# bernardomig/torch_semantic_segmentation

Hardware: AMD Instinct MI355X
Metric: images/sec (train step) fastscnn 1024x2048 bs=8 (higher is better)
Workload: dtype bf16; 1 GPU; fastscnn train step (zero_grad+fwd+CE(ignore 255)+bwd+AdamW), 8 x 3 x 1024 x 2048 per GPU, 19 classes, random-init weights; global_batch=8, parallelism=dp1, hip_graph=True, syncbn=False

## Files before the change

include/tss_hip.h:

```cpp
#ifndef TSS_HIP_H
#define TSS_HIP_H

#ifdef __cplusplus
extern "C" {
#endif

#define TSS_OK 0
#define TSS_ERR_DTYPE (-1)
#define TSS_ERR_SHAPE (-2)
#define TSS_ERR_ALIGN (-3)
#define TSS_ERR_HIP (-4)

#define TSS_F32 0
#define TSS_BF16 1

typedef struct tss_bn_bwd_job {
  const double* bstats; double count; const float* invstd; const float* gamma; int training; int accumulate;
  float* dgamma; float* dbeta; float* ga; float* gb; float* gce; int C;
  int xchg_world; int xchg_rank; void* xchg_peers[8]; void* xchg_counters;
} tss_bn_bwd_job;

enum {
  TSS_K_PWCONV_FWD = 0, TSS_K_PWCONV_BWD_DATA, TSS_K_PWCONV_BWD_WEIGHT,
  TSS_K_CONV3X3_FWD, TSS_K_CONV3X3_BWD_DATA, TSS_K_CONV3X3_BWD_WEIGHT,
// ... 158 lines not shown
int tss_mul_addrows_bwd(const void* g, long ldg, const void* u, long ldu, const void* a, long lda, void* du, long lddu, void* da,
                        long ldda, void* dr, long lddr, float* ws, int B, long HW, int C, int dtype, void* stream);
int tss_scale_rows(const void* x, long ldx, const float* m, void* out, long ldo, int B, long HW, int C, int dtype, void* stream);
int tss_cat2_add(const void* gl, long ldl, const void* gr, long ldr, const void* gs, long lds, void* out, long ldo, long P, int half,
                 int dtype, void* stream);
int tss_pad_channels(const void* g, long ldg, int C, void* out, long ldo, int CP, long P, int dtype, void* stream);
int tss_ssnbt_tail_fwd(const void* left, long ldl, const float* mean_l, const float* scale_l, const float* shift_l,
                       const void* right, long ldr, const float* mean_r, const float* scale_r, const float* shift_r,
                       const void* x, long ldx, const float* m, void* out, long ldo, int B, long HW, int C, int dtype, void* stream);
int tss_ssnbt_tail_bwd(const void* dout, long lddo, const void* out, long ldo,
                       const void* left, long ldl, const float* mean_l, const void* right, long ldr, const float* mean_r,
                       const float* m, void* e, long lde, void* gs, long ldgs, double* stats_l, double* stats_r,
                       int B, long HW, int C, int dtype, void* stream);

int tss_channel_shuffle(const void* x, long ldx, void* y, long ldy, long P, int C, int groups, int dtype, void* stream);

int tss_stem3x3_fwd(const void* x_nchw, int x_is_f32, const float* w, void* y, long ldy, double* stats,
                    int B, int Cin, int Hin, int Win, int N, int stride, int dtype, void* stream);
int tss_stem3x3_bwd_weight(const void* e, long lde, const void* yraw, long ldyr,
                           const float* ga, const float* gb, const float* gce, const float* gmu,
                           const void* x_nchw, int x_is_f32, float* dw,
                           float* ws ,
                           int B, int Cin, int Hin, int Win, int N, int stride, int dtype, void* stream);

int tss_dwconv3x3_fwd(const void* x, long ldx, const float* in_mean, const float* in_scale, const float* in_bias, int in_relu,
                      const float* w, void* y, long ldy, double* stats,
                      int B, int Hin, int Win, int C, int stride, int dil, int dtype, void* stream);
int tss_dwconv3x3_bwd_data(const void* e, long lde, const void* yraw, long ldyr,
                           const float* ga, const float* gb, const float* gce, const float* gmu, const float* w,
                           const void* xraw, long ldx, const float* in_mean, const float* in_scale, const float* in_bias, int in_relu,
                           void* e_in, long ldei, double* bstats, const float* wg_ws, float* wg_dw,
                           int B, int Hin, int Win, int C, int stride, int dil, int dtype, void* stream);
int tss_pwconv_bwd_data_radd_supported(long P, int K, int N, int dtype);
int tss_pwconv_bwd_data_joined(const void* e, long lde, const void* yraw, long ldyr,
                               const float* ga, const float* gb, const float* gce, const float* gmu, const float* w, const void* wT_bf16,
                               void* e_in, long ldei, const float* wg_ws, float* wg_dw, long wg_P, int wg_K, int wg_N,
                               const void* radd, long ldr, const void* join_out, long ldjo, const void* join_y, long ldjy,
                               const float* join_mean, double* join_bstats, long P, int K, int N, int dtype, void* stream);
int tss_pwconv_bwd_data_radd(const void* e, long lde, const void* yraw, long ldyr,
                             const float* ga, const float* gb, const float* gce, const float* gmu, const float* w, const void* wT_bf16,
                             void* e_in, long ldei, const float* wg_ws, float* wg_dw, long wg_P, int wg_K, int wg_N,
                             const void* radd, long ldr, long P, int K, int N, int dtype, void* stream);
int tss_pwconv_bwd_fused_preferred(long P, int Cin, int Cout, int dtype);
int tss_pwconv_bwd_fused_rows(long P, int Cin, int Cout);
int tss_pwconv_bwd_fused(const void* e, long lde, const void* yraw, long ldyr, const float* ga, const float* gb, const float* gce,
                         const float* gmu, const float* w, const void* wT_bf16, const void* x, long ldx, const float* in_mean,
// ... 270 lines not shown
```

torch_semantic_segmentation_amd/csrc/prof.cpp:

```cpp
#include <mutex>
#include <vector>

#include "common.h"

namespace {

struct KernelInfo { const char* name; const char* symbol; };
const KernelInfo kInfo[TSS_K_COUNT] = {
    {"pwconv_fwd", "pwfast_kernel<false>|pwfast_mc_kernel<false>|convgemm_kernel"},
    {"pwconv_bwd_data", "pwfast_kernel<true>|pwfast_mc_kernel<true>|pwbwd_kernel|pwsweep_kernel|convgemm_kernel"},
    {"pwconv_bwd_weight", "wgfast_kernel|wgrad_kernel"},
    {"conv3x3_fwd", "conv3x3_wstat_kernel|conv3x3_stream_kernel|conv3x3_lean_kernel<false>|fc1d_kernel|convgemm_kernel<fwd>"}, {"conv3x3_bwd_data", "conv3x3_lean_kernel<true>|fc1d_kernel|convgemm_kernel<bwd>"}, {"conv3x3_bwd_weight", "fc1d_wgrad_kernel|wgrad_kernel"},
    {"stem3x3_fwd", "stem_fwd_mfma_kernel|convgemm_kernel"}, {"stem3x3_bwd_weight", "stem_wgrad_mfma_kernel|stem_wgrad_kernel"},
    {"dwconv3x3_fwd", "dw_fwd_roll_kernel|dw_fwd_strip_kernel"}, {"dwconv3x3_bwd_data", "dw_bwd_roll_s1_kernel|dw_bwd_roll_s2_kernel|dw_bwd_data_strip_kernel"},
    {"dwconv3x3_bwd_weight", "dw_bwd_weight_strip_kernel"},
    {"bn_finalize", "bn_finalize_kernel"}, {"bn_bwd_finalize", "bn_bwd_finalize_kernel"},
    {"join_fwd", "join_fwd_kernel"}, {"join_bwd", "join_bwd_kernel"},
    {"dropout", "dropout_kernel"}, {"bias_grad", "colsum_kernel"}, {"adamw", "adamw_kernel"},
    {"bilinear_nhwc_fwd", "bilinear_nhwc_fwd_kernel|ppm_concat_fwd_kernel"}, {"bilinear_nhwc_bwd_rows", "bilinear_nhwc_bwd_rows_kernel|ppm_concat_bwd_kernel"},
    {"bilinear_nhwc_bwd_cols", "bilinear_nhwc_bwd_cols_kernel"},
    {"bilinear_planar_fwd", "bilinear_planar_fwd_kernel"},
    {"upsample_head_fwd", "upsample_head_fwd_kernel"}, {"upsample_head_bwd_rows", "upsample_head_bwd_rows_kernel"},
    {"upsample_head_bwd_cols", "upsample_head_bwd_cols_kernel"},
    {"adaptive_pool_fwd", "adaptive_pool_fwd_kernel|ppm_pool_fwd_kernel"}, {"adaptive_pool_bwd", "adaptive_pool_bwd_kernel|ppm_pool_bwd_kernel"},
    {"copy_nhwc", "copy_nhwc_kernel"},
    {"cross_entropy_fwd", "ce_fwd_kernel"}, {"cross_entropy_bwd", "ce_bwd_kernel"}, {"argmax_confusion", "argmax_confusion_kernel"},
    {"upsample_ce_fwd", "upsample_ce_onepass_kernel"}, {"upsample_ce_bwd", "upsample_ce_gather_kernel"},
    {"resize_flip_planar", "resize_flip_planar_kernel"}, {"multiscale_argmax_confusion", "multiscale_argmax_kernel"},
    {"sgd", "sgd_kernel"}, {"grad_norm", "grad_sqnorm_kernel|grad_sqnorm_final_kernel"},
    {"upsample_ce_wide_fwd", "wide_ce_kernel"}, {"upsample_ce_wide_bwd", "wide_ce_gather_kernel"},
    {"argmax_confusion_wide", "wide_upsample_argmax_kernel|wide_planar_argmax_kernel"},
    {"multiscale_argmax_confusion_wide", "wide_multiscale_argmax_kernel"},
};

struct Rec { int kid; hipEvent_t a, b; double bytes, flops; };
struct Total { long launches; double ms, bytes, flops; };
// ... 116 lines not shown
```

torch_semantic_segmentation_amd/csrc/stem.hip:

```cpp
#include "common.h"

namespace {

constexpr int NT = 256;

struct StemArgs {
  const void* x; int x_f32;
  const float* w; void* y; long ldy; double* stats;
  int B, Cin, Hin, Win, Hout, Wout, N, stride;
};

struct __attribute__((packed, aligned(4))) F4u { float x, y, z, w; };
template <typename TX>
__device__ __forceinline__ void stem_taps(const TX* x, long b, int oy, int ox, bool in, int Cin, int Hin, int Win,
                                          int stride, long plane, float v[27]) {
  if (sizeof(TX) == 4 && stride == 2 && Win >= 4) {
    const int ix0 = 2 * ox - 1;
    const int base = ix0 < 0 ? 0 : (ix0 > Win - 4 ? Win - 4 : ix0);
    const int sh = ix0 - base;
#pragma unroll
    for (int c = 0; c < 3; ++c)
#pragma unroll
      for (int ky = 0; ky < 3; ++ky) {
        const int iy = 2 * oy + ky - 1;
// ... 2 lines not shown
        const F4u f = *reinterpret_cast<const F4u*>(row);
#pragma unroll
        for (int kx = 0; kx < 3; ++kx) {
          const int idx = kx + sh;
          const float t = idx <= 0 ? f.x : (idx == 1 ? f.y : (idx == 2 ? f.z : f.w));
          v[c * 9 + ky * 3 + kx] = (vy && idx >= 0 && ix0 + kx < Win) ? t : 0.f;
        }
      }
    return;
  }
#pragma unroll
  for (int c = 0; c < 3; ++c)
#pragma unroll
    for (int ky = 0; ky < 3; ++ky) {
      const int iy = oy * stride + ky - 1;
      const bool vy = iy >= 0 && iy < Hin;
#pragma unroll
      for (int kx = 0; kx < 3; ++kx) {
        const int ix = ox * stride + kx - 1;
        const bool ok = in && c < Cin && vy && ix >= 0 && ix < Win;
        const long off = (b * Cin + (c < Cin ? c : 0)) * plane + (vy ? iy : 0) * (long)Win + (ix < 0 ? 0 : (ix >= Win ? Win - 1 : ix));
        const float t = (float)x[off];
        v[c * 9 + ky * 3 + kx] = ok ? t : 0.f;
      }
    }
}

template <typename TX>
__global__ __launch_bounds__(NT, 2) void stem_fwd_mfma_kernel(const StemArgs g) {
  typedef bf16_t T;
  constexpr int N = 32, TP = 256, PITCH = 40;
  __shared__ __align__(16) T Xp[TP * PITCH];
  __shared__ float red[NT / 64][2][N];
  const int tid = threadIdx.x, lane = tid & 63, wave = tid >> 6;
  const int fr = lane & 15, fq = lane >> 4;
  const int K = g.Cin * 9;
  bf16x8 wf[2];
#pragma unroll
  for (int i = 0; i < 2; ++i)
#pragma unroll
    for (int j = 0; j < 8; ++j) {
      const int k = fq * 8 + j;
      wf[i][j] = (T)(g.w[(i * 16 + fr) * K + (k < K ? k : 0)] * (k < K ? 1.f : 0.f));
    }
  const TX* x = reinterpret_cast<const TX*>(g.x);
  T* y = reinterpret_cast<T*>(g.y);
// ... 45 lines not shown
  if (g.stats) {
#pragma unroll
    for (int i = 0; i < 2; ++i)
#pragma unroll
      for (int q = 0; q < 4; ++q) {
        const float a = row16_sum(st1[i][q]), b = row16_sum(st2[i][q]);
        if (fr == 0) { red[wave][0][i * 16 + fq * 4 + q] = a; red[wave][1][i * 16 + fq * 4 + q] = b; }
      }
    __syncthreads();
    for (int i = tid; i < 2 * N; i += NT) {
      const int which = i / N, n = i - which * N;
      double s = 0.0;
      for (int wv = 0; wv < NT / 64; ++wv) s += (double)red[wv][which][n];
      g.stats[(long)blockIdx.x * 2 * N + i] = s;
      for (int r = blockIdx.x + gridDim.x; r < TSS_STAT_SLABS; r += gridDim.x) g.stats[(long)r * 2 * N + i] = 0.0;
    }
  }
}

struct StemWgradArgs {
  const void* e; long lde; const void* yraw; long ldyr; const float* ga; const float* gb; const float* gce; const float* gmu;
  const void* x; float* ws; float* dw;
  int B, Cin, Hin, Win, Hout, Wout, stride;
};

template <typename T, typename TX>
__global__ __launch_bounds__(NT, 2) void stem_wgrad_kernel(const StemWgradArgs g) {
  constexpr int N = 32, TP = 256, KP = 28;
  __shared__ __align__(16) float Gs[TP * N];
  __shared__ __align__(16) float Xs[TP * KP];
  const int tid = threadIdx.x;
  const T* e = reinterpret_cast<const T*>(g.e);
  const T* yr = reinterpret_cast<const T*>(g.yraw);
  const TX* x = reinterpret_cast<const TX*>(g.x);
  const int K = g.Cin * 9;
  const long P = (long)g.B * g.Hout * g.Wout;
  const long HWo = (long)g.Hout * g.Wout;
  const long plane = (long)g.Hin * g.Win;
  const long ntiles = (P + TP - 1) / TP;
  const int gcv = tid & 3;
  float ca[8], cb[8], cc[8], cm[8];
#pragma unroll
  for (int j = 0; j < 8; ++j) {
    ca[j] = g.ga ? g.ga[gcv * 8 + j] : 1.f;
    cb[j] = g.yraw ? g.gb[gcv * 8 + j] : 0.f;
    cc[j] = g.yraw ? g.gce[gcv * 8 + j] : 0.f;
// ... 151 lines not shown
      }
#pragma unroll
      for (int i = 0; i < 2; ++i)
#pragma unroll
        for (int j = 0; j < 2; ++j) acc[i][j] = __builtin_amdgcn_mfma_f32_16x16x32_bf16(gf[i], xf[j], acc[i][j], 0, 0, 0);
    }
  }
  __syncthreads();
  float* red = reinterpret_cast<float*>(Gt);
#pragma unroll
  for (int i = 0; i < 2; ++i)
#pragma unroll
    for (int j = 0; j < 2; ++j)
#pragma unroll
      for (int r = 0; r < 4; ++r) red[(wave * 32 + i * 16 + fq * 4 + r) * 32 + j * 16 + fr] = acc[i][j][r];
  __syncthreads();
  float* row = g.ws + (long)blockIdx.x * N * KP;
  for (int i = tid; i < N * KP; i += NT) {
    const int n = i / KP, k = i - n * KP;
    row[i] = red[n * 32 + k] + red[(32 + n) * 32 + k] + red[(64 + n) * 32 + k] + red[(96 + n) * 32 + k];
  }
}

__global__ __launch_bounds__(256) void stem_wgrad_reduce_kernel(const float* ws, float* dw, int K, int rows) {
  constexpr int N = 32, KP = 28;
  __shared__ float part[16][17];
  const int i = blockIdx.x * 16 + (threadIdx.x & 15);
  const int rg = threadIdx.x >> 4;
  float s = 0.f;
  if (i < N * KP) {
    for (int r0 = rg; r0 < rows; r0 += 16 * 8) {
      float v[8];
#pragma unroll
      for (int u = 0; u < 8; ++u) { const int r = r0 + 16 * u; v[u] = r < rows ? ws[(long)r * N * KP + i] : 0.f; }
#pragma unroll
      for (int u = 0; u < 8; ++u) s += v[u];
    }
  }
  part[rg][threadIdx.x & 15] = s;
  __syncthreads();
  if (threadIdx.x < 16 && i < N * KP) {
    const int n = i / KP, j = i - n * KP;
    if (j < K) {
      float t = 0.f;
#pragma unroll
      for (int q = 0; q < 16; ++q) t += part[q][threadIdx.x];
// ... 18 lines not shown
  return true;
}

bool tss_stem_direct_wgrad(const void* e, long lde, const void* yraw, long ldyr, const float* ga, const float* gb,
                           const float* gce, const float* gmu, const void* x_nchw, int x_is_f32, float* dw, float* ws,
                           int B, int Cin, int Hin, int Win, int N, int stride, int dtype, hipStream_t stream) {
  if (dtype != TSS_BF16 || Cin > 3 || N != 32 || !ws) return false;
  StemWgradArgs g = {};
  g.e = e; g.lde = lde; g.yraw = yraw; g.ldyr = ldyr; g.ga = ga; g.gb = gb; g.gce = gce; g.gmu = gmu;
  g.x = x_nchw; g.ws = ws; g.dw = dw;
  g.B = B; g.Cin = Cin; g.Hin = Hin; g.Win = Win; g.stride = stride;
  g.Hout = (Hin - 1) / stride + 1; g.Wout = (Win - 1) / stride + 1;
  const long P = (long)B * g.Hout * g.Wout;
  long grid = (P + 255) / 256;
  if (grid > TSS_STAT_SLABS) grid = TSS_STAT_SLABS;
  if (yraw && ga && gb && gce && gmu) {
    if (x_is_f32) hipLaunchKernelGGL((stem_wgrad_mfma_kernel<float>), dim3((int)grid), dim3(NT), 0, stream, g);
    else hipLaunchKernelGGL((stem_wgrad_mfma_kernel<bf16_t>), dim3((int)grid), dim3(NT), 0, stream, g);
  } else if (x_is_f32) hipLaunchKernelGGL((stem_wgrad_kernel<bf16_t, float>), dim3((int)grid), dim3(NT), 0, stream, g);
  else hipLaunchKernelGGL((stem_wgrad_kernel<bf16_t, bf16_t>), dim3((int)grid), dim3(NT), 0, stream, g);
  hipLaunchKernelGGL(stem_wgrad_reduce_kernel, dim3((32 * 28 + 15) / 16), dim3(256), 0, stream, ws, dw, Cin * 9, (int)grid);
  return true;
}
```

torch_semantic_segmentation_amd/csrc/wgrad.hip:

```cpp
#include "common.h"
#include "wgreduce.h"
#include "bnfin.h"

extern int g_tss_disable_fast;

namespace {

constexpr int TN = 128, TK = 128, NT = 256;
enum { A_PW = 0, A_TAPS = 1, A_STEM = 2 };

template <typename T> struct WMma;
template <> struct WMma<bf16_t> {
  static constexpr int PT = 64, KSTEP = 32;
  typedef bf16x8 Frag;
  static __device__ __forceinline__ Frag ld(const unsigned char* row, int swz, int ks, int q) {
    return *reinterpret_cast<const bf16x8*>(row + (((ks * 4 + q) ^ swz) << 4));
  }
  static __device__ __forceinline__ f32x4 mma(Frag a, Frag b, f32x4 c) {
    return __builtin_amdgcn_mfma_f32_16x16x32_bf16(a, b, c, 0, 0, 0);
  }
};
template <> struct WMma<float> {
  static constexpr int PT = 32, KSTEP = 4;
  typedef float Frag;
// ... 535 lines not shown
int launch(WgradArgs& g, int dtype, int kernel_id, hipStream_t stream, double alg_bytes) {
  if (g.P <= 0) return TSS_OK;
  const int nchn = (g.ND + TN - 1) / TN, nchk = (g.KD + TK - 1) / TK;
  const int tiles = nchn * nchk * g.ntaps;
  const int PT = dtype == TSS_BF16 ? WMma<bf16_t>::PT : WMma<float>::PT;
  const long nstage = (g.P + PT - 1) / PT;
  constexpr long MIN_STAGES = 8;
  long ns = 1024 / tiles;
  if (ns < 1) ns = 1;
  if (ns > (nstage + MIN_STAGES - 1) / MIN_STAGES) ns = (nstage + MIN_STAGES - 1) / MIN_STAGES;
  if (ns < 1) ns = 1;
  g.nsplit = (int)ns;
  const int grid = tiles * (int)ns;
  tss::ProfScope prof(kernel_id, stream, alg_bytes, 2.0 * (double)g.P * g.ND * g.KD * g.ntaps);
  TSS_WITH_DTYPE(dtype, hipLaunchKernelGGL(wgrad_kernel<TT>, dim3(grid), dim3(NT), 0, stream, g));
  return tss::check_last("wgrad");
}

}

bool tss_stem_direct_wgrad(const void* e, long lde, const void* yraw, long ldyr, const float* ga, const float* gb,
                           const float* gce, const float* gmu, const void* x_nchw, int x_is_f32, float* dw, float* ws,
                           int B, int Cin, int Hin, int Win, int N, int stride, int dtype, hipStream_t stream);

void tss_wg_reduce_standalone(const float* ws, float* dw, long P, int K, int N, hipStream_t stream) {
  const tss_wg::ReduceArgs r = reduce_args(ws, dw, P, K, N);
  hipLaunchKernelGGL(wg_reduce_kernel, dim3(r.nred), dim3(NT), 0, stream, r);
}

extern "C" {

int tss_pwconv_bwd_weight(const void* e, long lde, const void* yraw, long ldyr,
                          const float* ga, const float* gb, const float* gce, const float* gmu,
                          const void* xraw, long ldx, const float* in_mean, const float* in_scale, const float* in_bias, int in_relu,
                          float* dw, float* ws, int defer_reduce, long P, int K, int N, int dtype, const tss_bn_bwd_job* fin,
                          void* stream) {
  TSS_CHECK_DTYPE(dtype);
  TSS_REQUIRE(!fin || (fin->C > 0 && fin->count >= 1.0 && fin->bstats && fin->invstd && fin->ga && fin->gb && fin->gce), TSS_ERR_SHAPE);
  TSS_REQUIRE(K > 0 && N > 0 && (K % 8) == 0 && (lde % 8) == 0 && lde >= (N + 7) / 8 * 8 && (ldx % 8) == 0 && ldx >= K, TSS_ERR_SHAPE);
  TSS_REQUIRE(!yraw || ((ldyr % 8) == 0 && ldyr >= (N + 7) / 8 * 8 && ga && gb && gce && gmu), TSS_ERR_SHAPE);
  TSS_REQUIRE(tss::aligned16(e) && tss::aligned16(xraw), TSS_ERR_ALIGN);
  WgradArgs g = {};
  g.P = P; g.ND = N; g.KD = K; g.ntaps = 1; g.mode = A_PW;
  g.e = e; g.lde = lde; g.yraw = yraw; g.ldyr = ldyr; g.ga = ga; g.gb = gb; g.gce = gce; g.gmu = gmu;
  g.x = xraw; g.ldx = ldx; g.xm = in_mean; g.xs = in_scale; g.xb = in_bias; g.x_relu = in_relu;
  g.Hout = 1; g.Wout = 1;
// ... 90 lines not shown
                           const float* ga, const float* gb, const float* gce, const float* gmu,
                           const void* x_nchw, int x_is_f32, float* dw, float* ws,
                           int B, int Cin, int Hin, int Win, int N, int stride, int dtype, void* stream) {
  TSS_CHECK_DTYPE(dtype);
  TSS_REQUIRE(Cin >= 1 && Cin * 9 <= TK && N > 0 && (N % 8) == 0 && (lde % 8) == 0 && lde >= N, TSS_ERR_SHAPE);
  TSS_REQUIRE(!yraw || ((ldyr % 8) == 0 && ldyr >= N && ga && gb && gce && gmu), TSS_ERR_SHAPE);
  WgradArgs g = {};
  g.Hin = Hin; g.Win = Win; g.stride = stride; g.dil = 1; g.Cin = Cin;
  g.Hout = (Hin - 1) / stride + 1; g.Wout = (Win - 1) / stride + 1;
  g.P = (long)B * g.Hout * g.Wout; g.ND = N; g.KD = Cin * 9; g.ntaps = 1; g.mode = A_STEM;
  g.e = e; g.lde = lde; g.yraw = yraw; g.ldyr = ldyr; g.ga = ga; g.gb = gb; g.gce = gce; g.gmu = gmu;
  g.x = x_nchw; g.x_f32 = x_is_f32;
  g.dw = dw; g.drs = (long)Cin * 9; g.dcs = 1; g.dts = 0;
  const double bytes = (double)g.P * N * (yraw ? 2 : 1) * tss::esz(dtype) + (double)B * Cin * Hin * Win * (x_is_f32 ? 4 : tss::esz(dtype));
  if (dtype == TSS_BF16 && !g_tss_disable_fast && Cin <= 3 && N == 32 && ws) {
    tss::ProfScope prof(TSS_K_STEM_BWD_WEIGHT, (hipStream_t)stream, bytes, 2.0 * (double)g.P * N * Cin * 9);
    if (tss_stem_direct_wgrad(e, lde, yraw, ldyr, ga, gb, gce, gmu, x_nchw, x_is_f32, dw, ws, B, Cin, Hin, Win, N, stride,
                              dtype, (hipStream_t)stream))
      return tss::check_last("stem_direct_wgrad");
  }
  return launch(g, dtype, TSS_K_STEM_BWD_WEIGHT, (hipStream_t)stream, bytes);
}

#ifdef TSS_TIMING
int tss_debug_wg_timing(unsigned long long* out8, int reset) {
  if (hipMemcpyFromSymbol(out8, HIP_SYMBOL(g_wg_timing), sizeof(unsigned long long) * 8) != hipSuccess) return -1;
  if (reset) { unsigned long long z[8] = {0}; (void)hipMemcpyToSymbol(HIP_SYMBOL(g_wg_timing), z, sizeof(z)); }
  return 0;
}
#endif

}
```

torch_semantic_segmentation_amd/ops.py:

```python
import collections
import ctypes
import math
import os
import threading

import torch
from torch.autograd import Function
from torch.nn.modules.batchnorm import _BatchNorm

from . import _native as N

call, ptr, stream = N.call, N.ptr, N.stream



_DIRECT = [False]


class direct_grads:

    def __init__(self, enabled=True):
        self.enabled = bool(enabled)

    def __enter__(self):
        self.prev = _DIRECT[0]
        _DIRECT[0] = self.enabled
        return self

    def __exit__(self, *exc):
        _DIRECT[0] = self.prev
        return False


overlap_wgrad = os.environ.get('TSS_OVERLAP_WGRAD', '0') == '1'
fuse_dw_backward = os.environ.get('TSS_FUSE_DW_BWD', '0') == '1'
overlap_max_elems = int(os.environ.get('TSS_OVERLAP_MAX', str(48 << 20)))
overlap_min_elems = int(os.environ.get('TSS_OVERLAP_MIN', '0'))
batch_dw_reductions = os.environ.get('TSS_BATCH_DW_REDUCE', '1') == '1'
fuse_pw_backward = os.environ.get('TSS_PW_BWD_FUSED', '1') != '0'
sweep_pw_backward = os.environ.get('TSS_PW_SWEEP', '1') != '0'
postpone_wgrad = os.environ.get('TSS_POSTPONE_WGRAD', '1') != '0'
unfold_1d_wgrad = os.environ.get('TSS_FC1D_WGRAD', '1') != '0'
_CONST_ROWS = {}


def _per_device(cache, dev, make, stale=lambda got: False):
    key = (dev.type, dev.index)
    if key not in cache or stale(cache[key]):
        cache[key] = make()
    return cache[key]


def _const_rows(dev, n):
    m = max(768, n)
    return _per_device(_CONST_ROWS, dev, lambda: (torch.ones(m, dtype=torch.float32, device=dev), torch.zeros(m, dtype=torch.float32, device=dev)),
                       stale=lambda got: got[0].numel() < n)
_overlap_depth = [0]
postpone_in_overlap = os.environ.get('TSS_POSTPONE_OVERLAPPED', '0') == '1'


class _Pass:
    __slots__ = ('dw', 'wg', 'red')

    def __init__(self):
        self.dw = []
# ... 627 lines not shown
    dist.all_reduce(vec, op=dist.ReduceOp.SUM, group=group)
    return vec


def as_deferred(x):
    if isinstance(x, Deferred):
        return x
    _check_device(x)
    N.dtype_code(x.dtype)
    return Deferred(to_nhwc(x))


def materialize(d, relu_override=None):
    if not isinstance(d, Deferred):
        return d
    if d.link is None and not d.relu:
        return d.raw
    return join(d, None, d.relu)



class UnitCfg:
    __slots__ = ('kind', 'stride', 'dil', 'in_link', 'in_relu', 'bn', 'training', 'out_dtype', 'out_link',
                 'image_f32', 'cin', 'cout', 'params', 'res_fork', 'stash_fork', 'overlapped', 'kh', 'kw', 'drop_p', 'prev_join')


def _classify(conv, x_is_image):
    k = conv.kernel_size
    if tuple(k) in ((1, 3), (3, 1)):
        ax = 0 if tuple(k) == (1, 3) else 1
        d = conv.dilation[1 - ax]
        want_pad, want_dil = ((0, d), (1, d)) if ax == 0 else ((d, 0), (d, 1))
        if (conv.padding_mode != 'zeros' or conv.groups != 1 or tuple(conv.stride) != (1, 1) or tuple(conv.padding) != want_pad
                or tuple(conv.dilation) != want_dil or x_is_image):
            raise NotImplementedError('HIP path: 1x3 / 3x1 convolutions must be dense, stride 1, padding = dilation on the '
                                      'kernel axis: %r' % conv)
        return 'dense1d_w' if ax == 0 else 'dense1d_h', 1, d
    kh, kw = k
    if conv.groups == 1 and not x_is_image and kh % 2 == 1 and kw % 2 == 1 and (kh != kw or kh > 3):
        dd = [conv.dilation[i] for i in (0, 1) if k[i] > 1]
        d = dd[0]
        if (conv.padding_mode != 'zeros' or conv.stride[0] != conv.stride[1] or any(v != d for v in dd)
                or tuple(conv.padding) != (d * (kh - 1) // 2 if kh > 1 else 0, d * (kw - 1) // 2 if kw > 1 else 0)):
            raise NotImplementedError('HIP path: dense k x k convolutions need padding = dilation * (k - 1) / 2 and one stride: %r' % conv)
        return 'ckk', conv.stride[0], d
    if conv.padding_mode != 'zeros' or k[0] != k[1] or conv.stride[0] != conv.stride[1] \
            or conv.dilation[0] != conv.dilation[1] or conv.padding[0] != conv.padding[1]:
# ... 21 lines not shown


def drop_conv_supported(x, conv, p):
    if not (fuse_dropout and fuse_dropout_conv) or N.fast_paths_disabled() or not (0.0 < p < 1.0):
        return False
    try:
        kind = _classify(conv, False)[0]
    except NotImplementedError:
        return False
    raw = x.raw if isinstance(x, Deferred) else x
    if kind != 'pw' or raw.dim() != 4 or raw.dtype != torch.bfloat16 or raw.shape[1] != conv.in_channels:
        return False
    P, dt = npix(raw), N.dtype_code(raw.dtype)
    return bool(N.lib().tss_pwconv_drop_supported(P, conv.in_channels, conv.out_channels, dt)
                and N.lib().tss_pwconv_bwd_fused_drop_supported(P, conv.in_channels, conv.out_channels, dt))


def conv_unit(x, conv, bn=None, relu=False, out_dtype=None, weight=None, bias=_KEEP, gamma=None, beta=None, cout=None, drop_p=0.0):
    is_image = (not isinstance(x, Deferred)) and x.dim() == 4 and x.shape[1] % 8 != 0
    kind, stride, dil = _classify(conv, is_image)
    cfg = UnitCfg()
    cfg.kind, cfg.stride, cfg.dil = kind, stride, dil
    cfg.drop_p = float(drop_p)
    if cfg.drop_p and (kind != 'pw' or bn is not None):
        raise RuntimeError('conv_unit: dropout on load needs a 1x1 convolution without BatchNorm (drop_conv_supported)')
    cfg.overlapped = _overlap_depth[0] > 0 and not postpone_in_overlap
    cfg.cin, cfg.cout = conv.in_channels, (cout or conv.out_channels)
    cfg.kh, cfg.kw = conv.kernel_size
    if kind == 'stem':
        _check_device(x)
        if x.dtype not in (torch.float32, torch.bfloat16):
            raise TypeError('image must be float32 or bfloat16')
        x_raw = x.contiguous()
        cfg.in_link, cfg.in_relu = None, False
        cfg.image_f32 = x_raw.dtype == torch.float32
        cfg.out_dtype = out_dtype or x_raw.dtype
        cfg.res_fork = cfg.stash_fork = cfg.prev_join = None
    else:
        d = as_deferred(x).take()
        x_raw = d.raw
        cfg.in_link, cfg.in_relu = d.link, d.relu
        cfg.image_f32 = False
        cfg.out_dtype = x_raw.dtype
        cfg.res_fork = _take(x_raw, _FORK)
        cfg.stash_fork = _take(x_raw, _STASH)
        cfg.prev_join = cfg.res_fork.prev_join if cfg.res_fork is not None else (_take_join(x_raw) if d.link is None and not d.relu else None)
# ... 212 lines not shown
            link.mean, link.invstd, link.scale = pre.unbind(0)
        else:
            rbuf = _F32Buffers(bn, True)
            call('tss_bn_eval_affine', ptr(gamma), ptr(rbuf.mean), ptr(rbuf.var),
                 float(bn.eps), ptr(link.mean), ptr(link.invstd), ptr(link.scale), Cout, st)


def _frozen_link(bn, C, P, dev, st):
    gamma, beta = _f32(bn.weight), _f32(bn.bias)
    link = BNLink(C, P, False, gamma, beta, dev, slabs=False)
    _finalize_forward(link, bn, False, P, C, gamma, st)
    return link, beta


_FwdArgs = collections.namedtuple('_FwdArgs', 'cfg x weight bias y aff stats B Hin Win Cout P s d dt dev st')


def _fwd_stem(f):
    cfg, y = f.cfg, f.y
    if f.bias is not None:
        raise NotImplementedError('HIP path: stem convolution with bias')
    call('tss_stem3x3_fwd', ptr(f.x), int(cfg.image_f32), ptr(f.weight), ptr(y), ld(y), f.stats,
         f.B, cfg.cin, f.Hin, f.Win, f.Cout, f.s, f.dt, f.st)


def _fwd_pw(f):
    cfg, x, weight, y, st = f.cfg, f.x, f.weight, f.y, f.st
    if not cfg.drop_p:
        call('tss_pwconv_fwd', ptr(x), ld(x), *f.aff, int(cfg.in_relu), ptr(weight), _shadow(weight, 0), ptr(f.bias),
             ptr(y), ld(y), f.stats, f.P, cfg.cin, f.Cout, f.dt, st)
        return None
    mask = torch.empty((f.P, 16), dtype=torch.uint8, device=f.dev)
    counter = _dropout_counter(f.dev)
    call('tss_dropout_mask', ptr(counter), ptr(mask), f.P, cfg.cin, cfg.drop_p, st)
    if _drop_mask_probe is not None:
        _drop_mask_probe.append(mask)
    call('tss_pwconv_fwd_drop', ptr(x), ld(x), *f.aff, int(cfg.in_relu), ptr(weight), _shadow(weight, 0), ptr(f.bias),
         ptr(y), ld(y), ptr(mask), cfg.drop_p, ptr(counter), f.P, cfg.cin, f.Cout, f.dt, st)
    return mask


def _fwd_dw(f):
    cfg, x, y = f.cfg, f.x, f.y
    if f.bias is not None:
        raise NotImplementedError('HIP path: depthwise convolution with bias')
    call('tss_dwconv3x3_fwd', ptr(x), ld(x), *f.aff, int(cfg.in_relu), ptr(f.weight),
# ... 55 lines not shown


_NO_EXTRAS = (None, False, None)


def _wgrad_side_stream(cfg, need_dx, drop_mask, P, dev):
    if (overlap_wgrad and need_dx and cfg.kind != 'stem' and drop_mask is None
            and overlap_min_elems <= P * (cfg.cin + cfg.cout) <= overlap_max_elems):
        return _side_stream(dev)
    return None


def _new_e_in(c):
    if c.need_dx or c.drop_mask is not None:
        return new_nhwc(c.B, c.Cin, c.Hin, c.Win, c.e.dtype, c.dev)
    return None


def _res_grad(cfg):
    fork = cfg.res_fork
    return fork, (fork.g2 if fork is not None else None)


def _bwd_stem(c):
    ws = c.tmp((N.stat_slabs(), c.Cout * 28))
    call('tss_stem3x3_bwd_weight', *c.gargs, ptr(c.x), int(c.cfg.image_f32), ptr(c.dw), ptr(ws),
         c.B, c.Cin, c.Hin, c.Win, c.Cout, c.s, c.dt, c.st)
    if c.need_dx:
        raise NotImplementedError('HIP path: gradient with respect to the input image is not implemented')
    return None, _NO_EXTRAS



def _bwd_pw(c):
    P, Cin, Cout, dt = c.P, c.Cin, c.Cout, c.dt
    fused = bool(fuse_pw_backward and c.need_dx and c.side is None and c.e.dtype == torch.bfloat16
                 and not N.fast_paths_disabled() and N.lib().tss_pwconv_bwd_fused_preferred(P, Cin, Cout, dt))
    if c.drop_mask is not None:
        fused = True
    if fused:
        return _bwd_pw_fused(c)
    radd_s = _res_grad(c.cfg)[1]
    sweep = bool(sweep_pw_backward and c.need_dx and c.side is None and c.e.dtype == torch.bfloat16 and c.x.dtype == torch.bfloat16
                 and not N.fast_paths_disabled()
                 and N.lib().tss_pwconv_bwd_sweep_preferred(P, Cin, Cout, int(bool(c.deferred_in)), dt)
                 and (radd_s is None or (not c.deferred_in and radd_s.dtype == c.e.dtype and tuple(radd_s.shape) == tuple(c.x.shape)
                                         and is_nhwc(radd_s))))
    if sweep:
        return _bwd_pw_sweep(c)
    return _bwd_pw_split(c)
# ... 2357 lines not shown
```

Before: 1722 images/sec.

## Recompute stem conv output in weight-grad kernel instead of reading stored activation

Adds a stem weight-gradient kernel that recomputes the raw conv output on the fly with an MFMA from the image taps and weights, instead of reading the stored pre-BN output. This removes one full-resolution activation read in backward. It also prefetches the next tile's gradient and image taps into registers, using vector float4 loads for fp32 stride-2 input. It is guarded by a weight-version check and an environment flag. In exchange it spends extra MFMA work per tile and rounds the recomputed output to bf16, which may differ slightly from the stored values.

```diff
diff --git a/include/tss_hip.h b/include/tss_hip.h
--- a/include/tss_hip.h
+++ b/include/tss_hip.h
@@ -204,6 +204,10 @@
                            const void* x_nchw, int x_is_f32, float* dw,
                            float* ws ,
                            int B, int Cin, int Hin, int Win, int N, int stride, int dtype, void* stream);
+int tss_stem3x3_bwd_weight_rc(const void* e, long lde, const float* w,
+                              const float* ga, const float* gb, const float* gce, const float* gmu,
+                              const void* x_nchw, int x_is_f32, float* dw, float* ws,
+                              int B, int Cin, int Hin, int Win, int N, int stride, int dtype, void* stream);
 
 int tss_dwconv3x3_fwd(const void* x, long ldx, const float* in_mean, const float* in_scale, const float* in_bias, int in_relu,
                       const float* w, void* y, long ldy, double* stats,
diff --git a/torch_semantic_segmentation_amd/csrc/prof.cpp b/torch_semantic_segmentation_amd/csrc/prof.cpp
--- a/torch_semantic_segmentation_amd/csrc/prof.cpp
+++ b/torch_semantic_segmentation_amd/csrc/prof.cpp
@@ -11,7 +11,7 @@
     {"pwconv_bwd_data", "pwfast_kernel<true>|pwfast_mc_kernel<true>|pwbwd_kernel|pwsweep_kernel|convgemm_kernel"},
     {"pwconv_bwd_weight", "wgfast_kernel|wgrad_kernel"},
     {"conv3x3_fwd", "conv3x3_wstat_kernel|conv3x3_stream_kernel|conv3x3_lean_kernel<false>|fc1d_kernel|convgemm_kernel<fwd>"}, {"conv3x3_bwd_data", "conv3x3_lean_kernel<true>|fc1d_kernel|convgemm_kernel<bwd>"}, {"conv3x3_bwd_weight", "fc1d_wgrad_kernel|wgrad_kernel"},
-    {"stem3x3_fwd", "stem_fwd_mfma_kernel|convgemm_kernel"}, {"stem3x3_bwd_weight", "stem_wgrad_mfma_kernel|stem_wgrad_kernel"},
+    {"stem3x3_fwd", "stem_fwd_mfma_kernel|convgemm_kernel"}, {"stem3x3_bwd_weight", "stem_wgrad_rc_mfma_kernel|stem_wgrad_mfma_kernel|stem_wgrad_kernel"},
     {"dwconv3x3_fwd", "dw_fwd_roll_kernel|dw_fwd_strip_kernel"}, {"dwconv3x3_bwd_data", "dw_bwd_roll_s1_kernel|dw_bwd_roll_s2_kernel|dw_bwd_data_strip_kernel"},
     {"dwconv3x3_bwd_weight", "dw_bwd_weight_strip_kernel"},
     {"bn_finalize", "bn_finalize_kernel"}, {"bn_bwd_finalize", "bn_bwd_finalize_kernel"},
diff --git a/torch_semantic_segmentation_amd/csrc/stem.hip b/torch_semantic_segmentation_amd/csrc/stem.hip
--- a/torch_semantic_segmentation_amd/csrc/stem.hip
+++ b/torch_semantic_segmentation_amd/csrc/stem.hip
@@ -48,6 +48,79 @@
         const long off = (b * Cin + (c < Cin ? c : 0)) * plane + (vy ? iy : 0) * (long)Win + (ix < 0 ? 0 : (ix >= Win ? Win - 1 : ix));
         const float t = (float)x[off];
         v[c * 9 + ky * 3 + kx] = ok ? t : 0.f;
+      }
+    }
+}
+
+typedef float f32x4_a4 __attribute__((ext_vector_type(4), aligned(4)));
+template <typename TX, bool VEC> struct StemRaw { f32x4 f[VEC ? 9 : 1]; TX t[VEC ? 1 : 27]; int oy, ox; bool in; };
+template <typename TX, bool VEC>
+__device__ __forceinline__ void stem_taps_issue(const TX* x, long b, int oy, int ox, bool in, int Cin, int Hin, int Win, int stride,
+                                                long plane, StemRaw<TX, VEC>& r) {
+  r.oy = oy; r.ox = ox; r.in = in;
+  if constexpr (VEC) {
+    const int ix0 = 2 * ox - 1;
+    const int base = ix0 < 0 ? 0 : (ix0 > Win - 4 ? Win - 4 : ix0);
+#pragma unroll
+    for (int c = 0; c < 3; ++c)
+#pragma unroll
+      for (int ky = 0; ky < 3; ++ky) {
+        const int iy = 2 * oy + ky - 1;
+        const bool vy = c < Cin && iy >= 0 && iy < Hin;
+        const float* row = reinterpret_cast<const float*>(x) + (b * Cin + (c < Cin ? c : 0)) * plane + (long)(vy ? iy : 0) * Win + base;
+        r.f[c * 3 + ky] = *reinterpret_cast<const f32x4_a4*>(row);
+      }
+    return;
+  }
+#pragma unroll
+  for (int c = 0; c < 3; ++c)
+#pragma unroll
+    for (int ky = 0; ky < 3; ++ky) {
+      const int iy = oy * stride + ky - 1;
+      const bool vy = iy >= 0 && iy < Hin;
+#pragma unroll
+      for (int kx = 0; kx < 3; ++kx) {
+        const int ix = ox * stride + kx - 1;
+        const long off = (b * Cin + (c < Cin ? c : 0)) * plane + (vy ? iy : 0) * (long)Win + (ix < 0 ? 0 : (ix >= Win ? Win - 1 : ix));
+        r.t[c * 9 + ky * 3 + kx] = x[off];
+      }
+    }
+}
+template <typename TX, bool VEC>
+__device__ __forceinline__ void stem_taps_select(const StemRaw<TX, VEC>& r, int Cin, int Hin, int Win, int stride, float v[27]) {
+  const int oy = r.oy, ox = r.ox;
+  const bool in = r.in;
+  if constexpr (VEC) {
+    const int ix0 = 2 * ox - 1;
+    const int base = ix0 < 0 ? 0 : (ix0 > Win - 4 ? Win - 4 : ix0);
+    const int sh = ix0 - base;
+#pragma unroll
+    for (int c = 0; c < 3; ++c)
+#pragma unroll
+      for (int ky = 0; ky < 3; ++ky) {
+        const int iy = 2 * oy + ky - 1;
+        const bool vy = in && c < Cin && iy >= 0 && iy < Hin;
+        const f32x4 f = r.f[c * 3 + ky];
+#pragma unroll
+        for (int kx = 0; kx < 3; ++kx) {
+          const int idx = kx + sh;
+          const float t = idx <= 0 ? f[0] : (idx == 1 ? f[1] : (idx == 2 ? f[2] : f[3]));
+          v[c * 9 + ky * 3 + kx] = (vy && idx >= 0 && ix0 + kx < Win) ? t : 0.f;
+        }
+      }
+    return;
+  }
+#pragma unroll
+  for (int c = 0; c < 3; ++c)
+#pragma unroll
+    for (int ky = 0; ky < 3; ++ky) {
+      const int iy = oy * stride + ky - 1;
+      const bool vy = iy >= 0 && iy < Hin;
+#pragma unroll
+      for (int kx = 0; kx < 3; ++kx) {
+        const int ix = ox * stride + kx - 1;
+        const bool ok = in && c < Cin && vy && ix >= 0 && ix < Win;
+        v[c * 9 + ky * 3 + kx] = ok ? (float)r.t[c * 9 + ky * 3 + kx] : 0.f;
       }
     }
 }
@@ -139,6 +212,7 @@
   const void* e; long lde; const void* yraw; long ldyr; const float* ga; const float* gb; const float* gce; const float* gmu;
   const void* x; float* ws; float* dw;
   int B, Cin, Hin, Win, Hout, Wout, stride;
+  const float* w;
 };
 
 template <typename T, typename TX>
@@ -336,6 +410,145 @@
   }
 }
 
+__device__ __forceinline__ void wave_lds_sync() {
+  __builtin_amdgcn_fence(__ATOMIC_RELEASE, "wavefront");
+  __builtin_amdgcn_wave_barrier();
+  __builtin_amdgcn_fence(__ATOMIC_ACQUIRE, "wavefront");
+}
+
+template <typename TX, bool VEC>
+__global__ __launch_bounds__(NT, 2) void stem_wgrad_rc_mfma_kernel(const StemWgradArgs g) {
+  typedef bf16_t T;
+  constexpr int N = 32, TP = 256, KP = 28, ROW = TP + 8, PITCH = 40;
+  __shared__ __align__(16) T Gt[N * ROW];
+  __shared__ __align__(16) T Xt[32 * ROW];
+  __shared__ __align__(16) T Xp[TP * PITCH];
+  const int tid = threadIdx.x, lane = tid & 63, wave = tid >> 6;
+  const int fr = lane & 15, fq = lane >> 4;
+  const T* e = reinterpret_cast<const T*>(g.e);
+  const TX* x = reinterpret_cast<const TX*>(g.x);
+  const int K = g.Cin * 9;
+  const long P = (long)g.B * g.Hout * g.Wout;
+  const long HWo = (long)g.Hout * g.Wout;
+  const long plane = (long)g.Hin * g.Win;
+  const long ntiles = (P + TP - 1) / TP;
+  bf16x8 wf[2];
+#pragma unroll
+  for (int i = 0; i < 2; ++i)
+#pragma unroll
+    for (int j = 0; j < 8; ++j) {
+      const int k = fq * 8 + j;
+      const int n = (fr >> 2) * 8 + i * 4 + (fr & 3);
+      wf[i][j] = (T)(g.w[n * K + (k < K ? k : 0)] * (k < K ? 1.f : 0.f));
+    }
+  for (int i = tid; i < 5 * ROW; i += NT) Xt[27 * ROW + i] = (T)0.f;
+  float ca[8], cb[8], cc[8];
+  {
+    float v0[8], v1[8], v2[8], v3[8];
+#pragma unroll
+    for (int h = 0; h < 8; h += 4) {
+      V4<float>::load(g.ga + fq * 8 + h, v0 + h); V4<float>::load(g.gb + fq * 8 + h, v1 + h);
+      V4<float>::load(g.gce + fq * 8 + h, v2 + h); V4<float>::load(g.gmu + fq * 8 + h, v3 + h);
+    }
+#pragma unroll
+    for (int j = 0; j < 8; ++j) { ca[j] = v0[j]; cb[j] = v1[j]; cc[j] = -(v0[j] * v2[j]) - v1[j] * v3[j]; }
+  }
+  f32x4 acc[2][2];
+#pragma unroll
+  for (int i = 0; i < 2; ++i)
+#pragma unroll
+    for (int j = 0; j < 2; ++j) acc[i][j] = (f32x4){0.f, 0.f, 0.f, 0.f};
+  __syncthreads();
+
+  StemRaw<TX, VEC> raw;
+  uint4 rn[4];
+  auto issue = [&](long tile) __attribute__((always_inline)) {
+    const long p0 = tile * TP;
+#pragma unroll
+    for (int m = 0; m < 4; ++m) {
+      const long p = p0 + wave * 64 + m * 16 + fr;
+      const long pc = p < P ? p : 0;
+      rn[m] = *reinterpret_cast<const uint4*>(e + pc * g.lde + fq * 8);
+    }
+    const long p = p0 + tid;
+    const bool in = p < P;
+    const long pc = in ? p : 0;
+    const long b = pc / HWo; const long rem = pc - b * HWo;
+    const int oy = (int)(rem / g.Wout), ox = (int)(rem - (long)oy * g.Wout);
+    stem_taps_issue<TX, VEC>(x, b, oy, ox, in, g.Cin, g.Hin, g.Win, g.stride, plane, raw);
+  };
+  if ((long)blockIdx.x < ntiles) issue(blockIdx.x);
+
+  for (long tile = blockIdx.x; tile < ntiles; tile += gridDim.x) {
+    const long p0 = tile * TP;
+    wave_lds_sync();
+    uint4 re[4];
+    {
+      float v[32];
+      stem_taps_select<TX, VEC>(raw, g.Cin, g.Hin, g.Win, g.stride, v);
+#pragma unroll
+      for (int k = 27; k < 32; ++k) v[k] = 0.f;
+#pragma unroll
+      for (int k = 0; k < 27; ++k) Xt[k * ROW + tid] = (T)v[k];
+#pragma unroll
+      for (int h = 0; h < 4; ++h) V8<T>::store(Xp + tid * PITCH + h * 8, v + h * 8);
+#pragma unroll
+      for (int m = 0; m < 4; ++m) re[m] = rn[m];
+    }
+    if (tile + gridDim.x < ntiles) issue(tile + gridDim.x);
+    wave_lds_sync();
+#pragma unroll
+    for (int m = 0; m < 4; ++m) {
+      const int prow = wave * 64 + m * 16 + fr;
+      const bf16x8 xf = *reinterpret_cast<const bf16x8*>(Xp + prow * PITCH + fq * 8);
+      const bool in = p0 + prow < P;
+      const uint32_t* ue = reinterpret_cast<const uint32_t*>(&re[m]);
+#pragma unroll
+      for (int i = 0; i < 2; ++i) {
+        const f32x4 d = __builtin_amdgcn_mfma_f32_16x16x32_bf16(wf[i], xf, (f32x4){0.f, 0.f, 0.f, 0.f}, 0, 0, 0);
+#pragma unroll
+        for (int h = 0; h < 2; ++h) {
+          const int c = i * 4 + 2 * h;
+          const float ylo = (float)(T)d[2 * h], yhi = (float)(T)d[2 * h + 1];
+          const float lo = ca[c] * __uint_as_float(ue[c >> 1] << 16) + (cb[c] * ylo + cc[c]);
+          const float hi = ca[c + 1] * __uint_as_float(ue[c >> 1] & 0xffff0000u) + (cb[c + 1] * yhi + cc[c + 1]);
+          Gt[(fq * 8 + c) * ROW + prow] = (T)(in ? lo : 0.f);
+          Gt[(fq * 8 + c + 1) * ROW + prow] = (T)(in ? hi : 0.f);
+        }
+      }
+    }
+    wave_lds_sync();
+#pragma unroll
+    for (int ks = 0; ks < 2; ++ks) {
+      const int col = wave * 64 + ks * 32 + fq * 8;
+      bf16x8 gf[2], xf[2];
+#pragma unroll
+      for (int i = 0; i < 2; ++i) {
+        gf[i] = *reinterpret_cast<const bf16x8*>(Gt + (i * 16 + fr) * ROW + col);
+        xf[i] = *reinterpret_cast<const bf16x8*>(Xt + (i * 16 + fr) * ROW + col);
+      }
+#pragma unroll
+      for (int i = 0; i < 2; ++i)
+#pragma unroll
+        for (int j = 0; j < 2; ++j) acc[i][j] = __builtin_amdgcn_mfma_f32_16x16x32_bf16(gf[i], xf[j], acc[i][j], 0, 0, 0);
+    }
+  }
+  __syncthreads();
+  float* red = reinterpret_cast<float*>(Gt);
+#pragma unroll
+  for (int i = 0; i < 2; ++i)
+#pragma unroll
+    for (int j = 0; j < 2; ++j)
+#pragma unroll
+      for (int r = 0; r < 4; ++r) red[(wave * 32 + i * 16 + fq * 4 + r) * 32 + j * 16 + fr] = acc[i][j][r];
+  __syncthreads();
+  float* row = g.ws + (long)blockIdx.x * N * KP;
+  for (int i = tid; i < N * KP; i += NT) {
+    const int n = i / KP, k = i - n * KP;
+    row[i] = red[n * 32 + k] + red[(32 + n) * 32 + k] + red[(64 + n) * 32 + k] + red[(96 + n) * 32 + k];
+  }
+}
+
 __global__ __launch_bounds__(256) void stem_wgrad_reduce_kernel(const float* ws, float* dw, int K, int rows) {
   constexpr int N = 32, KP = 28;
   __shared__ float part[16][17];
@@ -400,3 +613,22 @@
   hipLaunchKernelGGL(stem_wgrad_reduce_kernel, dim3((32 * 28 + 15) / 16), dim3(256), 0, stream, ws, dw, Cin * 9, (int)grid);
   return true;
 }
+
+bool tss_stem_direct_wgrad_rc(const void* e, long lde, const float* w, const float* ga, const float* gb,
+                              const float* gce, const float* gmu, const void* x_nchw, int x_is_f32, float* dw, float* ws,
+                              int B, int Cin, int Hin, int Win, int N, int stride, int dtype, hipStream_t stream) {
+  if (dtype != TSS_BF16 || Cin > 3 || N != 32 || !ws || !w || !ga || !gb || !gce || !gmu) return false;
+  StemWgradArgs g = {};
+  g.e = e; g.lde = lde; g.w = w; g.ga = ga; g.gb = gb; g.gce = gce; g.gmu = gmu;
+  g.x = x_nchw; g.ws = ws; g.dw = dw;
+  g.B = B; g.Cin = Cin; g.Hin = Hin; g.Win = Win; g.stride = stride;
+  g.Hout = (Hin - 1) / stride + 1; g.Wout = (Win - 1) / stride + 1;
+  const long P = (long)B * g.Hout * g.Wout;
+  long grid = (P + 255) / 256;
+  if (grid > TSS_STAT_SLABS) grid = TSS_STAT_SLABS;
+  if (x_is_f32 && stride == 2 && Win >= 4) hipLaunchKernelGGL((stem_wgrad_rc_mfma_kernel<float, true>), dim3((int)grid), dim3(NT), 0, stream, g);
+  else if (x_is_f32) hipLaunchKernelGGL((stem_wgrad_rc_mfma_kernel<float, false>), dim3((int)grid), dim3(NT), 0, stream, g);
+  else hipLaunchKernelGGL((stem_wgrad_rc_mfma_kernel<bf16_t, false>), dim3((int)grid), dim3(NT), 0, stream, g);
+  hipLaunchKernelGGL(stem_wgrad_reduce_kernel, dim3((32 * 28 + 15) / 16), dim3(256), 0, stream, ws, dw, Cin * 9, (int)grid);
+  return true;
+}
diff --git a/torch_semantic_segmentation_amd/csrc/wgrad.hip b/torch_semantic_segmentation_amd/csrc/wgrad.hip
--- a/torch_semantic_segmentation_amd/csrc/wgrad.hip
+++ b/torch_semantic_segmentation_amd/csrc/wgrad.hip
@@ -581,6 +581,9 @@
 bool tss_stem_direct_wgrad(const void* e, long lde, const void* yraw, long ldyr, const float* ga, const float* gb,
                            const float* gce, const float* gmu, const void* x_nchw, int x_is_f32, float* dw, float* ws,
                            int B, int Cin, int Hin, int Win, int N, int stride, int dtype, hipStream_t stream);
+bool tss_stem_direct_wgrad_rc(const void* e, long lde, const float* w, const float* ga, const float* gb,
+                              const float* gce, const float* gmu, const void* x_nchw, int x_is_f32, float* dw, float* ws,
+                              int B, int Cin, int Hin, int Win, int N, int stride, int dtype, hipStream_t stream);
 
 void tss_wg_reduce_standalone(const float* ws, float* dw, long P, int K, int N, hipStream_t stream) {
   const tss_wg::ReduceArgs r = reduce_args(ws, dw, P, K, N);
@@ -717,6 +720,23 @@
   return launch(g, dtype, TSS_K_STEM_BWD_WEIGHT, (hipStream_t)stream, bytes);
 }
 
+int tss_stem3x3_bwd_weight_rc(const void* e, long lde, const float* w,
+                              const float* ga, const float* gb, const float* gce, const float* gmu,
+                              const void* x_nchw, int x_is_f32, float* dw, float* ws,
+                              int B, int Cin, int Hin, int Win, int N, int stride, int dtype, void* stream) {
+  TSS_CHECK_DTYPE(dtype);
+  TSS_REQUIRE(dtype == TSS_BF16 && !g_tss_disable_fast && Cin >= 1 && Cin <= 3 && N == 32 && B >= 1 && Hin >= 1 && Win >= 1 &&
+              stride >= 1 && (lde % 8) == 0 && lde >= N && e && w && ga && gb && gce && gmu && x_nchw && dw && ws, TSS_ERR_SHAPE);
+  TSS_REQUIRE(tss::aligned16(e), TSS_ERR_ALIGN);
+  const long P = (long)B * ((Hin - 1) / stride + 1) * ((Win - 1) / stride + 1);
+  const double bytes = (double)P * N * tss::esz(dtype) + (double)B * Cin * Hin * Win * (x_is_f32 ? 4 : tss::esz(dtype));
+  tss::ProfScope prof(TSS_K_STEM_BWD_WEIGHT, (hipStream_t)stream, bytes, 2.0 * (double)P * N * Cin * 9);
+  if (!tss_stem_direct_wgrad_rc(e, lde, w, ga, gb, gce, gmu, x_nchw, x_is_f32, dw, ws, B, Cin, Hin, Win, N, stride, dtype,
+                                (hipStream_t)stream))
+    return TSS_ERR_SHAPE;
+  return tss::check_last("stem_direct_wgrad_rc");
+}
+
 #ifdef TSS_TIMING
 int tss_debug_wg_timing(unsigned long long* out8, int reset) {
   if (hipMemcpyFromSymbol(out8, HIP_SYMBOL(g_wg_timing), sizeof(unsigned long long) * 8) != hipSuccess) return -1;
diff --git a/torch_semantic_segmentation_amd/ops.py b/torch_semantic_segmentation_amd/ops.py
--- a/torch_semantic_segmentation_amd/ops.py
+++ b/torch_semantic_segmentation_amd/ops.py
@@ -41,6 +41,7 @@
 sweep_pw_backward = os.environ.get('TSS_PW_SWEEP', '1') != '0'
 postpone_wgrad = os.environ.get('TSS_POSTPONE_WGRAD', '1') != '0'
 unfold_1d_wgrad = os.environ.get('TSS_FC1D_WGRAD', '1') != '0'
+stem_wgrad_recompute = os.environ.get('TSS_STEM_WGRAD_RC', '1') != '0'
 _CONST_ROWS = {}
 
 
@@ -714,7 +715,8 @@
 
 class UnitCfg:
     __slots__ = ('kind', 'stride', 'dil', 'in_link', 'in_relu', 'bn', 'training', 'out_dtype', 'out_link',
-                 'image_f32', 'cin', 'cout', 'params', 'res_fork', 'stash_fork', 'overlapped', 'kh', 'kw', 'drop_p', 'prev_join')
+                 'image_f32', 'cin', 'cout', 'params', 'res_fork', 'stash_fork', 'overlapped', 'kh', 'kw', 'drop_p', 'prev_join',
+                 'stem_rc')
 
 
 def _classify(conv, x_is_image):
@@ -782,6 +784,7 @@
     cfg = UnitCfg()
     cfg.kind, cfg.stride, cfg.dil = kind, stride, dil
     cfg.drop_p = float(drop_p)
+    cfg.stem_rc = None
     if cfg.drop_p and (kind != 'pw' or bn is not None):
         raise RuntimeError('conv_unit: dropout on load needs a 1x1 convolution without BatchNorm (drop_conv_supported)')
     cfg.overlapped = _overlap_depth[0] > 0 and not postpone_in_overlap
@@ -1040,6 +1043,8 @@
         raise NotImplementedError('HIP path: stem convolution with bias')
     call('tss_stem3x3_fwd', ptr(f.x), int(cfg.image_f32), ptr(f.weight), ptr(y), ld(y), f.stats,
          f.B, cfg.cin, f.Hin, f.Win, f.Cout, f.s, f.dt, f.st)
+    if y.dtype == torch.bfloat16 and cfg.cin <= 3 and f.Cout == 32 and not N.fast_paths_disabled():
+        cfg.stem_rc = (f.weight, f.weight._version)
 
 
 def _fwd_pw(f):
@@ -1141,10 +1146,22 @@
     return fork, (fork.g2 if fork is not None else None)
 
 
+def _stem_recompute(c):
+    rc = c.cfg.stem_rc
+    return bool(stem_wgrad_recompute and rc is not None and c.y is not None and c.link is not None and c.link.training
+                and c.weight is rc[0] and c.weight._version == rc[1] and c.e.dtype == torch.bfloat16 and c.Cin <= 3 and c.Cout == 32
+                and not N.fast_paths_disabled())
+
+
 def _bwd_stem(c):
     ws = c.tmp((N.stat_slabs(), c.Cout * 28))
-    call('tss_stem3x3_bwd_weight', *c.gargs, ptr(c.x), int(c.cfg.image_f32), ptr(c.dw), ptr(ws),
-         c.B, c.Cin, c.Hin, c.Win, c.Cout, c.s, c.dt, c.st)
+    if _stem_recompute(c):
+        e, lde, _, _, ga, gb, gce, gmu = c.gargs
+        call('tss_stem3x3_bwd_weight_rc', e, lde, ptr(c.weight), ga, gb, gce, gmu, ptr(c.x), int(c.cfg.image_f32), ptr(c.dw), ptr(ws),
+             c.B, c.Cin, c.Hin, c.Win, c.Cout, c.s, c.dt, c.st)
+    else:
+        call('tss_stem3x3_bwd_weight', *c.gargs, ptr(c.x), int(c.cfg.image_f32), ptr(c.dw), ptr(ws),
+             c.B, c.Cin, c.Hin, c.Win, c.Cout, c.s, c.dt, c.st)
     if c.need_dx:
         raise NotImplementedError('HIP path: gradient with respect to the input image is not implemented')
     return None, _NO_EXTRAS
```

Result: faster. 1740 images/sec, median of 6 (+1.1%).
